# DLR-RM/AugmentedAutoencoder

Measured on NVIDIA H100. Metric: pose queries/sec (encode+codebook NN), higher is better.
Workload: dtype f32 via split-fp16 tensor-core products (3x, fp32 accumulate)

## Files before the change

### augmentedautoencoder_b200/csrc/tc_gemm.cu

```cuda
#include <limits.h>

#include <algorithm>
#include <vector>

#include "tc.cuh"
#include "tc_common.cuh"
#include "tc_plan.cuh"

namespace aae {

using namespace tc;

PFN_tmapEncodeTiled get_tmap_encoder() {
  static PFN_tmapEncodeTiled fn = nullptr;
  if (!fn) {
    void* p = nullptr;
    cudaDriverEntryPointQueryResult q;
    if (cudaGetDriverEntryPoint("cuTensorMapEncodeTiled", &p, cudaEnableDefault, &q) == cudaSuccess && q == cudaDriverEntryPointSuccess)
      fn = reinterpret_cast<PFN_tmapEncodeTiled>(p);
  }
  return fn;
}

int make_tmap_f16(CUtensorMap* out, const void* base, int rank, const uint64_t* dims, const uint64_t* strides_bytes, const uint32_t* box,
                  int swizzle_bytes) {
  PFN_tmapEncodeTiled enc = get_tmap_encoder();
  if (!enc) { set_error("cuTensorMapEncodeTiled is unavailable in this driver"); return AAE_ERR_CUDA; }
  cuuint64_t gdim[5], gstr[4];
  cuuint32_t bx[5], es[5];
  for (int i = 0; i < rank; ++i) { gdim[i] = dims[i]; bx[i] = box[i]; es[i] = 1; }
  for (int i = 0; i + 1 < rank; ++i) gstr[i] = strides_bytes[i];
  CUresult r = enc(out, CU_TENSOR_MAP_DATA_TYPE_FLOAT16, (cuuint32_t)rank, const_cast<void*>(base), gdim, gstr, bx, es,
                   CU_TENSOR_MAP_INTERLEAVE_NONE, swizzle_bytes == 64 ? CU_TENSOR_MAP_SWIZZLE_64B : CU_TENSOR_MAP_SWIZZLE_128B,
                   CU_TENSOR_MAP_L2_PROMOTION_L2_256B,
                   CU_TENSOR_MAP_FLOAT_OOB_FILL_NONE);
  if (r != CUDA_SUCCESS) { set_error("cuTensorMapEncodeTiled failed with CUresult %d (rank %d)", (int)r, rank); return AAE_ERR_CUDA; }
  return AAE_OK;
}

template <int N_TILE, int STAGES, int PLANES = 2>
struct TcSmem {
  static constexpr int A_BYTES = 128 * TC_KCH * 2;
  static constexpr int W_BYTES = N_TILE * TC_KCH * 2;
  static constexpr int STAGE_BYTES = PLANES * A_BYTES + PLANES * W_BYTES;
  static constexpr int BODY = STAGES * STAGE_BYTES;
  static constexpr int TOTAL = BODY + 1024  + 256 ;
};

struct TcTile {
  int m0, n0, z, it_begin, it_end;
};
template <int N_TILE>
__device__ __forceinline__ TcTile tc_tile(const TcGemmParams& p, const TcTiles& g, int t) {
  TcTile r;
  const int yz = t / g.n;
  const int y = yz % g.m;
  r.z = yz / g.m;
  r.m0 = y * 128;
  r.n0 = (t - yz * g.n) * N_TILE;
  r.it_begin = r.z * p.iters_per_split;
  r.it_end = min(p.taps * p.chunks_per_tap, r.it_begin + p.iters_per_split);
  return r;
}

template <int N_TILE, int STAGES, int PLANES = 2>
__global__ void __launch_bounds__(TC_THREADS, 1)
tc_gemm_kernel(const __grid_constant__ CUtensorMap tm_a_hi, const __grid_constant__ CUtensorMap tm_a_lo,
               const __grid_constant__ CUtensorMap tm_w_hi, const __grid_constant__ CUtensorMap tm_w_lo, const TcGemmParams p,
               const TcTiles tiles) {
  using S = TcSmem<N_TILE, STAGES, PLANES>;
  constexpr int R = N_TILE / 2;
  extern __shared__ uint8_t smem_raw[];
  uint8_t* smem = reinterpret_cast<uint8_t*>((reinterpret_cast<uintptr_t>(smem_raw) + 1023) & ~(uintptr_t)1023);
  uint64_t* full_bar = reinterpret_cast<uint64_t*>(smem + S::BODY);
  uint64_t* empty_bar = full_bar + STAGES;

  const int warp = threadIdx.x >> 5;
  const int lane = threadIdx.x & 31;

  if (threadIdx.x == 0) {
    prefetch_tmap(&tm_a_hi);
    if constexpr (PLANES == 2) prefetch_tmap(&tm_a_lo);
    prefetch_tmap(&tm_w_hi);
    if constexpr (PLANES == 2) prefetch_tmap(&tm_w_lo);
    for (int s = 0; s < STAGES; ++s) { mbar_init(&full_bar[s], 1); mbar_init(&empty_bar[s], 2); }
    fence_barrier_init();
  }
  __syncthreads();

  if (warp < 4) {
    setmaxnreg_dec<TC_PRODUCER_REGS>();
    if (warp == 0 && lane == 0) {
      const int hw = p.OH * p.OW;
      int i = 0;
      for (int t = blockIdx.x; t < tiles.count; t += gridDim.x) {
        const TcTile T = tc_tile<N_TILE>(p, tiles, t);
        const int b0 = T.m0 / hw, rem = T.m0 - b0 * hw;
        const int oh0 = rem / p.OW, ow0 = rem - oh0 * p.OW;
        for (int it = T.it_begin; it < T.it_end; ++it, ++i) {
          const int s = i % STAGES;
          const uint32_t ph = (uint32_t)(i / STAGES) & 1u;
          mbar_wait(&empty_bar[s], ph ^ 1u);
          const int tap = it / p.chunks_per_tap, cc = it - tap * p.chunks_per_tap;
          uint8_t* st = smem + s * S::STAGE_BYTES;
          mbar_arrive_expect_tx(&full_bar[s], S::STAGE_BYTES);
          const int c0 = p.tap_ch[tap] + cc * TC_KCH;
          const int x = ow0 + p.tap_dj[tap], y = oh0 + p.tap_di[tap];
          const int kcol = it * TC_KCH;
          tma_load_4d(st, &tm_a_hi, &full_bar[s], c0, x, y, b0);
          if constexpr (PLANES == 2) tma_load_4d(st + S::A_BYTES, &tm_a_lo, &full_bar[s], c0, x, y, b0);
          tma_load_2d(st + PLANES * S::A_BYTES, &tm_w_hi, &full_bar[s], kcol, T.n0);
          if constexpr (PLANES == 2) tma_load_2d(st + 2 * S::A_BYTES + S::W_BYTES, &tm_w_lo, &full_bar[s], kcol, T.n0);
        }
      }
    }
  } else {
    setmaxnreg_inc<TC_CONSUMER_REGS>();
    const int wg = (warp - 4) >> 2;
    const bool releases = (warp & 3) == 0 && lane == 0;
    constexpr int H = R / 8;
    float acc[R], crs[R], v[R];
#pragma unroll
    for (int j = 0; j < R; ++j) { acc[j] = 0.f; crs[j] = 0.f; v[j] = 0.f; }
    int pm0 = 0, pn0 = 0, pz = 0, half = 2;
    auto epilogue_half = [&](int h) {
      if (h == 0) tc_epilogue_frag<PLANES, 0, H>(p, v, pm0, pn0, pz, warp, lane);
      else tc_epilogue_frag<PLANES, H, 2 * H>(p, v, pm0, pn0, pz, warp, lane);
    };
    int i = 0;
    for (int t = blockIdx.x; t < tiles.count; t += gridDim.x) {
      const TcTile T = tc_tile<N_TILE>(p, tiles, t);
      for (int it = T.it_begin; it < T.it_end; ++it, ++i) {
        const int s = i % STAGES;
        mbar_wait(&full_bar[s], (uint32_t)(i / STAGES) & 1u);
        const uint32_t st = smem_u32(smem + s * S::STAGE_BYTES);
        const uint32_t a_off = (uint32_t)(wg * 64 * TC_KCH * 2);
        const uint64_t a_hi = make_sw128_kmajor_desc(st + a_off);
        const uint64_t a_lo = make_sw128_kmajor_desc(st + S::A_BYTES + a_off);
        const uint64_t w_hi = make_sw128_kmajor_desc(st + PLANES * S::A_BYTES);
        const uint64_t w_lo = make_sw128_kmajor_desc(st + 2 * S::A_BYTES + S::W_BYTES);
        wgmma_fence_regs(acc);
        if constexpr (PLANES == 2) wgmma_fence_regs(crs);
        wgmma_fence();
#pragma unroll
        for (int k = 0; k < TC_KCH / 16; ++k) {
          const uint32_t first = (it > T.it_begin || k > 0) ? 1u : 0u;
          Wgmma<N_TILE>::template ss<0, 0>(acc, desc_advance_k(a_hi, k), desc_advance_k(w_hi, k), first);
          if constexpr (PLANES == 2) {
            Wgmma<N_TILE>::template ss<0, 0>(crs, desc_advance_k(a_lo, k), desc_advance_k(w_hi, k), first);
            Wgmma<N_TILE>::template ss<0, 0>(crs, desc_advance_k(a_hi, k), desc_advance_k(w_lo, k), 1u);
          }
        }
        wgmma_commit();
        if (half < 2) epilogue_half(half++);
        wgmma_wait<1>();
        wgmma_fence_regs(acc);
        if constexpr (PLANES == 2) wgmma_fence_regs(crs);
        if (it > T.it_begin && releases) mbar_arrive(&empty_bar[(i - 1) % STAGES]);
      }
      wgmma_wait<0>();
      wgmma_fence_regs(acc);
      if constexpr (PLANES == 2) wgmma_fence_regs(crs);
      if (T.it_end > T.it_begin && releases) mbar_arrive(&empty_bar[(i - 1) % STAGES]);
      while (half < 2) epilogue_half(half++);
      tc_epilogue_values<PLANES>(p, acc, crs, T.it_end > T.it_begin, v);
      pm0 = T.m0 + wg * 64; pn0 = T.n0; pz = T.z; half = 0;
    }
    while (half < 2) epilogue_half(half++);
  }
}

namespace {

template <int PLANES>
__global__ void pack_weights_kernel(const float* __restrict__ w, int taps, int cin, int cout, float scale, __half* __restrict__ hi,
                                    __half* __restrict__ lo, unsigned* __restrict__ range_flag, unsigned range_bit) {
  __shared__ float tile[32][33];
  const int tap = blockIdx.z;
  const int ci0 = blockIdx.y * 32, co0 = blockIdx.x * 32;
  for (int i = threadIdx.y; i < 32; i += 8) {
    const int ci = ci0 + i, co = co0 + threadIdx.x;
    tile[i][threadIdx.x] = (ci < cin && co < cout) ? w[((long long)tap * cin + ci) * cout + co] : 0.f;
  }
  __syncthreads();
  for (int i = threadIdx.y; i < 32; i += 8) {
    const int co = co0 + i, ci = ci0 + threadIdx.x;
    if (co < cout && ci < cin)
      tc_store_f16<PLANES>(tile[threadIdx.x][i] * scale, hi, lo, (long long)co * taps * cin + (long long)tap * cin + ci, range_flag, range_bit);
  }
// ... 56 lines not shown
  return AAE_OK;
}

int TcPlanes::alloc(size_t n, int planes) {
  AAE_TRY(tc_dev_alloc((void**)&hi, n * sizeof(__half)));
  return planes == 2 ? tc_dev_alloc((void**)&lo, n * sizeof(__half)) : AAE_OK;
}

void TcPlanes::release() {
  cudaFree(hi);
  cudaFree(lo);
  hi = lo = nullptr;
}

int TcPlanes::encode(TcMaps& m, int rank, const uint64_t* dims, const uint64_t* strides_bytes, const uint32_t* box, int swizzle_bytes) const {
  AAE_TRY(make_tmap_f16(&m.hi, hi, rank, dims, strides_bytes, box, swizzle_bytes));
  if (lo == nullptr) {
    m.lo = m.hi;
    return AAE_OK;
  }
  return make_tmap_f16(&m.lo, lo, rank, dims, strides_bytes, box, swizzle_bytes);
}

constexpr int TC_STAGES_SPLIT = 3, TC_STAGES_FP16 = 6;
static_assert(TcSmem<TC_N_TILE, TC_STAGES_FP16, 1>::TOTAL == TcSmem<TC_N_TILE, TC_STAGES_SPLIT>::TOTAL, "same footprint");

int tc_launch_layer(const TcLayer& T, dim3 tiles, cudaStream_t s, int planes) {
  const long long count = (long long)tiles.x * tiles.y * tiles.z;
  AAE_REQUIRE(count <= INT_MAX, "tc_gemm: %lld tiles exceed the kernel's int tile index", count);
  int device = 0, sms = 0;
  AAE_CUDA_OK(cudaGetDevice(&device));
  AAE_CUDA_OK(cudaDeviceGetAttribute(&sms, cudaDevAttrMultiProcessorCount, device));
  const TcTiles g{(int)tiles.y, (int)tiles.x, (int)count};
  const unsigned ctas = (unsigned)std::min<long long>(count, sms);
  return with_planes(planes, [&](auto P) {
    constexpr int STAGES = P == 1 ? TC_STAGES_FP16 : TC_STAGES_SPLIT;
    using S = TcSmem<TC_N_TILE, STAGES, P>;
    auto kern = tc_gemm_kernel<TC_N_TILE, STAGES, P>;
    AAE_CUDA_OK(cudaFuncSetAttribute(kern, cudaFuncAttributeMaxDynamicSharedMemorySize, S::TOTAL));
    kern<<<ctas, TC_THREADS, S::TOTAL, s>>>(T.tm_a.hi, T.tm_a.lo, T.tm_w.hi, T.tm_w.lo, T.gp, g);
    AAE_LAUNCH_OK();
    return AAE_OK;
  });
}

int tc_encoder_create(int device, const aae_net_cfg* cfg, TcEncoder** out) {
  *out = nullptr;
  const int L = cfg->num_layers;
  AAE_REQUIRE(aae_device_supported(device), "AAE_PREC_TC_SPLIT needs a compute-capability 9.0 device (wgmma/TMA)");
  AAE_REQUIRE(L >= 2, "AAE_PREC_TC_SPLIT: at least two conv layers expected");
  const int planes = tc_planes(cfg->precision);
  if (planes == 1 && !tc_conv1_supported(cfg)) {
    set_error("AAE_PREC_TC_FP16: the first layer needs the tensor-core conv1 (128 x 128 x 3 crops, 128 filters, k = 5, stride 2)");
    return AAE_ERR_UNSUPPORTED;
  }
  TcEncoder* h = new TcEncoder();
  h->device = device;
  h->cfg = *cfg;
  h->planes = planes;
  int ih = (cfg->in_h + cfg->strides[0] - 1) / cfg->strides[0], iw = (cfg->in_w + cfg->strides[0] - 1) / cfg->strides[0], ic = cfg->filters[0];
  const int B = cfg->max_batch;
  int st = AAE_OK;
  for (int l = 1; l <= L && st == AAE_OK; ++l) {
// ... 3 lines not shown
    if (!dense) {
      if (cfg->strides[l] != 2 || cfg->kernel_size != 5 || (ih & 1) || (iw & 1) || ic % 64 != 0 || cfg->filters[l] % 32 != 0) {
        set_error("AAE_PREC_TC_SPLIT: layer %d unsupported (needs k=5, stride 2, even dims, Cin %% 64 == 0, Cout %% 32 == 0)", l);
        st = AAE_ERR_UNSUPPORTED;
        break;
      }
      T.in_h = ih; T.in_w = iw; T.in_c = ic;
      T.out_h = ih / 2; T.out_w = iw / 2; T.out_c = cfg->filters[l];
      T.taps = 25;
      if (!pow2(T.out_w) || !pow2(T.out_h) || T.out_w > 128) { set_error("AAE_PREC_TC_SPLIT: output dims must be powers of two <= 128"); st = AAE_ERR_UNSUPPORTED; break; }
      T.BW = T.out_w;
      T.BH = std::min(T.out_h, 128 / T.BW);
      T.BB = 128 / (T.BW * T.BH);
    } else {
      T.in_h = T.in_w = 1; T.in_c = ih * iw * ic;
      T.out_h = T.out_w = 1; T.out_c = cfg->latent;
      T.taps = 1; T.BW = 1; T.BH = 1; T.BB = 128;
      h->flat = T.in_c;
      if (T.in_c % 64 != 0 || T.out_c % 32 != 0) { set_error("AAE_PREC_TC_SPLIT: dense layer needs flat %% 64 == 0 and latent %% 32 == 0"); st = AAE_ERR_UNSUPPORTED; break; }
    }
    const int B_pad = (int)ceil_div(B, T.BB) * T.BB;
    if ((st = T.in.alloc((size_t)B_pad * T.in_h * T.in_w * T.in_c, planes)) != AAE_OK) break;
    if ((st = T.w.alloc((size_t)T.out_c * T.taps * T.in_c, planes)) != AAE_OK) break;
    if (!dense) {
      const uint64_t C4 = 4ull * T.in_c, W2 = T.in_w / 2, H2 = T.in_h / 2;
      const uint64_t dims[4] = {C4, W2, H2, (uint64_t)B_pad};
      const uint64_t strides[3] = {C4 * 2, W2 * C4 * 2, H2 * W2 * C4 * 2};
      const uint32_t box[4] = {(uint32_t)TC_KCH, (uint32_t)T.BW, (uint32_t)T.BH, (uint32_t)T.BB};
      if ((st = T.in.encode(T.tm_a, 4, dims, strides, box)) != AAE_OK) break;
    } else {
      const uint64_t dims[4] = {(uint64_t)T.in_c, 1, 1, (uint64_t)B_pad};
      const uint64_t strides[3] = {(uint64_t)T.in_c * 2, (uint64_t)T.in_c * 2, (uint64_t)T.in_c * 2};
      const uint32_t box[4] = {(uint32_t)TC_KCH, 1, 1, 128};
      if ((st = T.in.encode(T.tm_a, 4, dims, strides, box)) != AAE_OK) break;
    }
    {
      const uint64_t K = (uint64_t)T.taps * T.in_c;
      const uint64_t dims[2] = {K, (uint64_t)T.out_c};
      const uint64_t strides[1] = {K * 2};
      const uint32_t box[2] = {(uint32_t)TC_KCH, (uint32_t)std::min(TC_N_TILE, T.out_c)};
      if ((st = T.w.encode(T.tm_w, 2, dims, strides, box)) != AAE_OK) break;
    }
    TcGemmParams& g = T.gp;
    g.N = T.out_c; g.OH = T.out_h; g.OW = T.out_w; g.BW = T.BW; g.BH = T.BH;
    g.taps = T.taps; g.chunks_per_tap = T.in_c / TC_KCH;
    g.iters_per_split = g.taps * g.chunks_per_tap;
    for (int t = 0; t < T.taps; ++t) {
      if (dense) { g.tap_di[t] = 0; g.tap_dj[t] = 0; g.tap_ch[t] = 0; continue; }
      const int kh = t / 5, kw = t % 5;
      g.tap_di[t] = (int8_t)((kh + 1) / 2 - 1);
      g.tap_dj[t] = (int8_t)((kw + 1) / 2 - 1);
      g.tap_ch[t] = ((((kh + 1) & 1) << 1) | ((kw + 1) & 1)) * T.in_c;
    }
    g.unscale = 1.f / (ACT_SCALE * W_SCALE);
    g.out_scale = ACT_SCALE;
    g.relu = dense ? 0 : 1;
    h->layers.push_back(T);
    if (!dense) { ih = T.out_h; iw = T.out_w; ic = T.out_c; }
  }
  if (st == AAE_OK) {
    for (size_t i = 0; i + 1 < h->layers.size(); ++i) {
      TcGemmParams& g = h->layers[i].gp;
      g.out_hi = h->layers[i + 1].in.hi;
      g.out_lo = h->layers[i + 1].in.lo;
      g.out_mode = (i + 2 == h->layers.size()) ? OUT_PLAIN_SPLIT : OUT_S2D_SPLIT;
    }
    TcLayer& D = h->layers.back();
    const int total = D.gp.taps * D.gp.chunks_per_tap;
    h->dense_splits = std::min(total, 66);
    D.gp.iters_per_split = (total + h->dense_splits - 1) / h->dense_splits;
    h->dense_splits = (total + D.gp.iters_per_split - 1) / D.gp.iters_per_split;
    D.gp.out_mode = OUT_F32;
    st = dev_alloc((void**)&h->partials, (size_t)h->dense_splits * (B + 128) * cfg->latent * sizeof(float));
    D.gp.out_f32 = h->partials;
  }
  if (st == AAE_OK) st = dev_alloc((void**)&h->range_flag, sizeof(unsigned));
  if (st == AAE_OK)
    for (size_t i = 0; i + 1 < h->layers.size(); ++i) {
      h->layers[i].gp.range_flag = h->range_flag;
      h->layers[i].gp.range_bit = 1u << (i + 1);
    }
  if (st == AAE_OK && tc_conv1_supported(cfg)) st = tc_conv1_create(device, cfg, &h->conv1);
  if (st != AAE_OK) { tc_encoder_destroy(h); return st; }
  *out = h;
  return AAE_OK;
}

void tc_encoder_destroy(TcEncoder* h) {
  if (!h) return;
  for (auto& T : h->layers) { T.in.release(); T.w.release(); }
  cudaFree(h->partials);
  cudaFree(h->fwd_partials);
  cudaFree(h->dbg);
  if (h->owns_range_flag) cudaFree(h->range_flag);
// ... 62 lines not shown
    T.gp.M = dense ? B : B * T.out_h * T.out_w;
    dim3 grid((unsigned)ceil_div(T.gp.M, 128), (unsigned)ceil_div(T.out_c, TC_N_TILE), dense ? (unsigned)h->dense_splits : 1u);
    int splits = 1;
    if (!dense && T.gp.out_mode != OUT_F32) {
      const int tiles = (int)(grid.x * grid.y), total_iters = T.gp.taps * T.gp.chunks_per_tap;
      if (tiles * 2 <= 132) {
        splits = std::min(132 / tiles, std::max(1, total_iters / 24));
        const size_t per_split = (size_t)T.gp.M * T.gp.N;
        if (per_split * (size_t)splits > h->fwd_partial_floats) {
          const size_t want = std::min<size_t>(per_split * (size_t)splits, (size_t)32 << 20);
          if (want > h->fwd_partial_floats) {
            cudaFree(h->fwd_partials);
            h->fwd_partials = nullptr; h->fwd_partial_floats = 0;
            AAE_TRY(dev_alloc((void**)&h->fwd_partials, want * sizeof(float)));
            h->fwd_partial_floats = want;
          }
          splits = (int)std::min<size_t>((size_t)splits, h->fwd_partial_floats / per_split);
        }
        splits = std::max(splits, 1);
      }
    }
    if (splits > 1) {
      TcLayer S = T;
      const int total_iters = T.gp.taps * T.gp.chunks_per_tap;
      S.gp.iters_per_split = (int)ceil_div(total_iters, splits);
      splits = (int)ceil_div(total_iters, S.gp.iters_per_split);
      S.gp.out_mode = OUT_F32;
      S.gp.out_f32 = h->fwd_partials;
      grid.z = (unsigned)splits;
      AAE_TRY(tc_launch_layer(S, grid, s, h->planes));
      const long long groups = (long long)T.gp.M * (T.gp.N >> 3);
      const unsigned fin_grid = (unsigned)std::min<long long>(132 * 8, ceil_div(groups, 256));
      with_planes(h->planes, [&](auto P) { splitk_forward_finish_kernel<P><<<fin_grid, 256, 0, s>>>(h->fwd_partials, splits, T.gp); });
      AAE_LAUNCH_OK();
    } else {
      AAE_TRY(tc_launch_layer(T, grid, s, h->planes));
    }
    if (dense) AAE_TRY(launch_splitk_reduce(h->partials, h->dense_splits, (int64_t)B * cfg.latent, cfg.latent, dense_b, ACT_NONE, z_out, s));
    timer->mark(s);
  }
  return AAE_OK;
}

int tc_encoder_set_bias(TcEncoder* h, int layer, const float* bias_dev) {
  if (layer >= 1 && layer < (int)h->layers.size()) h->layers[layer - 1].gp.bias = bias_dev;
  return AAE_OK;
}

int tc_encoder_activation(TcEncoder* h, int layer, int B, const float** ptr, int64_t* count, cudaStream_t s) {
// ... 66 lines not shown
    }
    x[((b * 2 * h + 2 * i + (cls >> 1)) * (2LL * w) + 2 * j + (cls & 1)) * c + co] = 1.f / (1.f + expf(-s));
  }
}

__global__ void tile_bias_kernel(const float* __restrict__ b, int cout, float* __restrict__ out) {
  const int i = blockIdx.x * blockDim.x + threadIdx.x;
  if (i < 4 * cout) out[i] = b[i % cout];
}

}

int tc_layer_setup_plain(TcLayer& T, int B, int planes) {
  const int B_pad = (int)ceil_div(B, T.BB) * T.BB;
  const uint64_t K = (uint64_t)T.taps * T.in_c;
  const int rows = (int)ceil_div(T.gp.N, TC_N_TILE) * TC_N_TILE;
  AAE_TRY(T.in.alloc((size_t)B_pad * T.in_h * T.in_w * T.in_c, planes));
  AAE_TRY(T.w.alloc((size_t)rows * K, planes));
  {
    const uint64_t dims[4] = {(uint64_t)T.in_c, (uint64_t)T.in_w, (uint64_t)T.in_h, (uint64_t)B_pad};
    const uint64_t strides[3] = {(uint64_t)T.in_c * 2, (uint64_t)T.in_w * T.in_c * 2, (uint64_t)T.in_h * T.in_w * T.in_c * 2};
    const uint32_t box[4] = {(uint32_t)TC_KCH, (uint32_t)T.BW, (uint32_t)T.BH, (uint32_t)T.BB};
    AAE_TRY(T.in.encode(T.tm_a, 4, dims, strides, box));
  }
  const uint64_t dims[2] = {K, (uint64_t)rows};
  const uint64_t strides[1] = {K * 2};
  const uint32_t box[2] = {(uint32_t)TC_KCH, (uint32_t)TC_N_TILE};
  return T.w.encode(T.tm_w, 2, dims, strides, box);
}

int tc_decoder_create(int device, const aae_net_cfg* cfg, TcDecoder** out) {
  *out = nullptr;
  AAE_REQUIRE(aae_device_supported(device), "AAE_PREC_TC_SPLIT needs a compute-capability 9.0 device (wgmma/TMA)");
  const int L = cfg->num_layers;
  AAE_REQUIRE(cfg->kernel_size == 5 && cfg->in_h == cfg->in_w, "AAE_PREC_TC_SPLIT decoder: kernel 5, square crops");
  TcDecoder* h = new TcDecoder();
  h->device = device;
  h->cfg = *cfg;
  h->planes = tc_planes(cfg->precision);
  const int B = cfg->max_batch;
  int h0 = cfg->in_h;
  for (int i = 0; i < L; ++i) h0 /= 2;
  std::vector<int> nf(L);
  for (int i = 0; i < L; ++i) nf[i] = cfg->filters[L - 1 - i];
  int st = AAE_OK;
  for (int l = 0; l <= L && st == AAE_OK; ++l) {
// ... 8 lines not shown
    } else {
      const int hh = h0 << (l - 1);
      T.in_h = T.in_w = hh; T.in_c = nf[l - 1];
      const int cout = l < L ? nf[l] : cfg->in_c;
      T.out_h = T.out_w = 2 * hh; T.out_c = cout;
      T.taps = 9;
      if (hh > 128 || (hh & (hh - 1)) || T.in_c % 64 != 0 || (l < L && cout % 64 != 0)) {
        set_error("tc decoder: layer %d unsupported (power-of-two size <= 128, Cin %% 64, Cout %% 64)", l); st = AAE_ERR_UNSUPPORTED; break;
      }
      T.BW = hh; T.BH = std::min(hh, 128 / T.BW); T.BB = 128 / (T.BW * T.BH);
      g.OH = g.OW = hh;
      if (l < L) { g.N = 4 * cout; g.relu = 1; g.out_mode = OUT_D2S_SPLIT; }
      else {
        if (36 * cout > 128) {
          set_error("tc decoder: %d output channels, the tensor-core output layer takes at most 3 (AAE_PREC_FP32_SIMT takes any count)", cout);
          st = AAE_ERR_UNSUPPORTED; break;
        }
        T.taps = 1; g.N = 128; g.relu = 0; g.out_mode = OUT_F32;
        st = dev_alloc((void**)&h->out_p, (size_t)ceil_div((int64_t)B * hh * hh, 128) * 128 * 128 * sizeof(float));
        if (st != AAE_OK) break;
      }
    }
    g.BW = T.BW; g.BH = T.BH; g.taps = T.taps; g.chunks_per_tap = T.in_c / TC_KCH;
    g.iters_per_split = g.taps * g.chunks_per_tap;
    for (int t = 0; t < T.taps; ++t) {
      g.tap_di[t] = (int8_t)(T.taps == 1 ? 0 : t / 3 - 1);
      g.tap_dj[t] = (int8_t)(T.taps == 1 ? 0 : t % 3 - 1);
      g.tap_ch[t] = 0;
    }
    g.unscale = 1.f / (ACT_SCALE * W_SCALE);
    g.out_scale = ACT_SCALE;
    if ((st = tc_layer_setup_plain(T, B, h->planes)) != AAE_OK) { h->layers.push_back(T); break; }
    h->layers.push_back(T);
    float* bz = nullptr;
    if (l > 0 && l < L) st = dev_alloc((void**)&bz, (size_t)g.N * sizeof(float));
    h->bias_dev.push_back(bz);
    h->wm_floats = std::max(h->wm_floats, (size_t)9 * T.in_c * 4 * T.out_c);
  }
  if (st == AAE_OK) st = dev_alloc((void**)&h->wm_tmp, h->wm_floats * sizeof(float));
  if (st == AAE_OK) st = dev_alloc((void**)&h->range_flag, sizeof(unsigned));
  if (st == AAE_OK) {
    for (size_t i = 0; i + 1 < h->layers.size(); ++i) {
      h->layers[i].gp.out_hi = h->layers[i + 1].in.hi;
      h->layers[i].gp.out_lo = h->layers[i + 1].in.lo;
      h->layers[i].gp.range_flag = h->range_flag;
      h->layers[i].gp.range_bit = 1u << i;
    }
// ... 82 lines not shown
```

### augmentedautoencoder_b200/csrc/tc_plan.cuh

```cuda
#pragma once
#include <stdlib.h>

#include <type_traits>
#include <vector>

#include "tc.cuh"
#include "tc_common.cuh"

namespace aae {

enum TcOutMode : int {
  OUT_S2D_SPLIT = 0,
  OUT_PLAIN_SPLIT = 1,
  OUT_F32 = 2,
  OUT_D2S_SPLIT = 3
};

struct TcGemmParams {
  int M;
  int N;
  int OH, OW;
  int BW, BH;
  int taps;
  int chunks_per_tap;
  int iters_per_split;
  int8_t tap_di[32], tap_dj[32];
  int tap_ch[32];
  float unscale;
  const unsigned* amax_bits;
  float out_scale;
  const float* bias;
  int relu;
  int out_mode;
  __half* out_hi;
  __half* out_lo;
  float* out_f32;
  unsigned* range_flag;
  unsigned range_bit;
};

constexpr float TC_F16_OVERFLOW = 65520.f;



__host__ __device__ __forceinline__ int tc_dyn_exponent(unsigned amax_bits) {
  int e = (int)((amax_bits >> 23) & 0xffu) - 127;
  return e < -100 ? -100 : (e > 100 ? 100 : e);
}
__device__ __forceinline__ float tc_dyn_scale(unsigned amax_bits) { return __int_as_float((127 + 13 - tc_dyn_exponent(amax_bits)) << 23); }
__device__ __forceinline__ float tc_dyn_unscale(unsigned amax_bits) { return __int_as_float((127 - 13 + tc_dyn_exponent(amax_bits)) << 23); }

constexpr float ACT_SCALE = 16.f;
constexpr float W_SCALE = 256.f;
constexpr int TC_STAGES = 2;
constexpr int TC_THREADS = 384;
constexpr int TC_N_TILE = 128;
constexpr int TC_PRODUCER_REGS = 24, TC_CONSUMER_REGS = 240;
constexpr int TC_KCH = 64;

struct TcMaps {
  CUtensorMap hi, lo;
};

struct TcPlanes {
  __half* hi = nullptr;
  __half* lo = nullptr;
  int alloc(size_t n, int planes);
  void release();
  int encode(TcMaps& m, int rank, const uint64_t* dims, const uint64_t* strides_bytes, const uint32_t* box, int swizzle_bytes = 128) const;
};

template <class F>
auto with_planes(int planes, F&& f) {
  return planes == 1 ? f(std::integral_constant<int, 1>{}) : f(std::integral_constant<int, 2>{});
}

struct TcLayer {
  int in_h, in_w, in_c, out_h, out_w, out_c;
  int taps, BW, BH, BB;
  TcPlanes in;
  TcPlanes w;
  TcMaps tm_a, tm_w;
  TcGemmParams gp;
};

struct TcEncoder {
  int device;
  aae_net_cfg cfg;
  unsigned* range_flag = nullptr;
  bool owns_range_flag = true;
  std::vector<TcLayer> layers;
  int flat;
  float* partials = nullptr;
  float* fwd_partials = nullptr;
  size_t fwd_partial_floats = 0;
  int dense_splits = 1;
  TcConv1* conv1 = nullptr;
  int planes = 2;
  float* dbg = nullptr;
  size_t dbg_floats = 0;
};


struct TcDecoder {
  int device;
// ... 192 lines not shown
    for (int h = 0; h < 2; ++h) {
      const TcRow& r = rows[h];
      if (!r.valid) continue;
      float f[2] = {fmaxf(__fadd_rn(v[4 * j + 2 * h], b0), floor_v), fmaxf(__fadd_rn(v[4 * j + 2 * h + 1], b1), floor_v)};
      amax = fmaxf(amax, fmaxf(fabsf(f[0]), fabsf(f[1])));
      long long off = r.row_off + n;
      if (p.out_mode == OUT_D2S_SPLIT) {
        const int cls = n / cq, co = n - cls * cq;
        off = ((long long)(r.b * 2 * p.OH + 2 * r.i + (cls >> 1)) * (2 * p.OW) + 2 * r.j + (cls & 1)) * cq + co;
      }
      tc_store_f16<PLANES>(f, p.out_scale, p.out_hi, p.out_lo, off);
    }
  }
  if (p.range_flag != nullptr && !(amax * p.out_scale < TC_F16_OVERFLOW)) atomicOr(p.range_flag, p.range_bit);
}

struct TcTiles {
  int n, m, count;
};

int tc_launch_layer(const TcLayer& T, dim3 tiles, cudaStream_t s, int planes);
int tc_dev_alloc(void** p, size_t bytes);
int tc_layer_setup_plain(TcLayer& T, int B, int planes);

}
```

### augmentedautoencoder_b200/csrc/tc_train.cu

```cuda
#include <algorithm>
#include <vector>

#include "tc.cuh"
#include "tc_common.cuh"
#include "tc_plan.cuh"

namespace aae {

using namespace tc;

struct TcWgradParams {
  int cin_blocks;
  int OH, OW;
  int BWk, BHk;
  int chunks_per_image;
  int total_chunks;
  int chunks_per_split;
  int8_t tap_di[32], tap_dj[32];
  int tap_ch[32];
  int m_tiles;
  TcGemmParams ep;
};

template <int N_TILE, int STAGES, int PLANES = 2>
// ... 439 lines not shown
  AAE_REQUIRE(enc && dec && enc->conv1, "tensor-core trainer: needs the tensor-core encoder (incl. conv1) and decoder plans");
  AAE_REQUIRE(enc->planes == dec->planes, "tensor-core trainer: the encoder and decoder plans use different operand planes");
  TcTrainPlan* h = new TcTrainPlan();
  h->device = enc->device; h->max_batch = max_batch; h->enc = enc; h->dec = dec; h->planes = enc->planes;
  const int B = max_batch;
  int st = AAE_OK;
  const int Ld = (int)dec->layers.size() - 1;
  const int Le = (int)enc->layers.size() - 1;
  size_t raw_max = 0, part_max = 0, wm_max = 0;
  auto add_unit = [&](TcUnit& U, const TcLayer& F, int x_c_total) -> int {
    TcLayer& T = U.dg;
    memset(&T.gp, 0, sizeof(T.gp));
    T.in_h = U.gh; T.in_w = U.gw; T.in_c = U.gN;
    T.out_h = U.gh; T.out_w = U.gw; T.out_c = U.nd;
    T.taps = U.dg_taps;
    T.BW = U.gw; T.BH = std::min(U.gh, 128 / T.BW); T.BB = 128 / (T.BW * T.BH);
    if (U.gw > 128 || (U.gw & (U.gw - 1)) || (U.gh & (U.gh - 1)) || U.gN % TC_KCH != 0 || U.nd % TC_N_TILE != 0 || U.cin % 128 != 0 ||
        U.gN % 64 != 0 || (U.gh * U.gw) % 32 != 0) {
      set_error("tensor-core trainer: layer geometry unsupported (G %dx%dx%d, dgrad N %d, Cin %d)", U.gh, U.gw, U.gN, U.nd, U.cin);
      return AAE_ERR_UNSUPPORTED;
    }
    TcGemmParams& g = T.gp;
    g.N = U.nd; g.OH = U.gh; g.OW = U.gw; g.BW = T.BW; g.BH = T.BH;
    g.taps = T.taps; g.chunks_per_tap = U.gN / TC_KCH; g.iters_per_split = g.taps * g.chunks_per_tap;
    for (int t = 0; t < T.taps; ++t) {
      g.tap_di[t] = (int8_t)(T.taps == 1 ? 0 : t / 3 - 1);
      g.tap_dj[t] = (int8_t)(T.taps == 1 ? 0 : t % 3 - 1);
      g.tap_ch[t] = 0;
    }
    g.unscale = 1.f / W_SCALE;
    g.out_mode = OUT_F32;
    AAE_TRY(tc_layer_setup_plain(T, B, h->planes));
    U.x = F.in;
    const int x_bpad = (int)ceil_div(B, F.BB) * F.BB, g_bpad = (int)ceil_div(B, T.BB) * T.BB;
    AAE_TRY(make_wgrad_maps(U, x_c_total, x_bpad, g_bpad));
    for (int t = 0; t < U.taps_w; ++t) { U.wp.tap_di[t] = F.gp.tap_di[t]; U.wp.tap_dj[t] = F.gp.tap_dj[t]; U.wp.tap_ch[t] = F.gp.tap_ch[t]; }
    raw_max = std::max(raw_max, (size_t)B * U.gh * U.gw * U.nd);
    wm_max = std::max(wm_max, (size_t)U.taps_w * U.cin * U.gN);
    return AAE_OK;
  };
  for (int l = Ld; l >= 1 && st == AAE_OK; --l) {
    const TcLayer& F = dec->layers[l];
    TcUnit U;
    U.enc = false; U.cin = F.in_c; U.cout = F.out_c;
    U.gh = F.in_h; U.gw = F.in_w;
    U.sep = l == Ld;
    U.gN = U.sep ? 128 : 4 * F.out_c;
// ... 139 lines not shown

int tc_train_conv1_wgrad(TcTrainPlan* h, const float* x_dev, int B, float* dw_out, cudaStream_t s) {
  TcUnit& U = h->units[h->c1];
  const aae_net_cfg& cfg = h->enc->cfg;
  const long long pixels = (long long)B * U.gh * U.gw;
  const int pad_t = std::max((U.gh - 1) * 2 + 5 - cfg.in_h, 0) / 2, pad_l = std::max((U.gw - 1) * 2 + 5 - cfg.in_w, 0) / 2;
  with_planes(h->planes, [&](auto P) {
    conv1_im2col_kernel<P><<<ew_grid(pixels * 16), 256, 0, s>>>(x_dev, pixels, cfg.in_h, cfg.in_w, U.gh, U.gw, pad_t, pad_l, ACT_SCALE, h->c1_x.hi,
                                                                h->c1_x.lo);
  });
  AAE_LAUNCH_OK();
  AAE_REQUIRE((size_t)128 * U.gN <= h->wm_floats, "tc trainer: scratch too small for the conv1 wgrad");
  AAE_TRY(tc_train_unit_wgrad(h, h->c1, B, h->wm, s));
  AAE_CUDA_OK(cudaMemcpyAsync(dw_out, h->wm, (size_t)75 * U.gN * sizeof(float), cudaMemcpyDeviceToDevice, s));
  return AAE_OK;
}

int tc_train_unit_dgrad(TcTrainPlan* h, int u, int B, cudaStream_t s) {
  TcUnit& U = h->units[u];
  TcLayer& T = U.dg;
  T.gp.M = B * U.gh * U.gw;
  T.gp.amax_bits = h->amax + u;
  const int m_tiles = (int)ceil_div(T.gp.M, 128), n_tiles = U.nd / TC_N_TILE;
  const int total_iters = T.gp.taps * T.gp.chunks_per_tap;
  int splits = std::max(1, 132 / std::max(1, m_tiles * n_tiles));
  splits = std::min(splits, std::max(1, total_iters / 64));
  const long long mn = (long long)T.gp.M * U.nd;
  if ((size_t)splits * (size_t)mn > h->partial_floats) splits = 1;
  T.gp.iters_per_split = (int)ceil_div(total_iters, splits);
  splits = (int)ceil_div(total_iters, T.gp.iters_per_split);
  T.gp.out_f32 = splits > 1 ? h->partials : h->raw;
  dim3 grid((unsigned)m_tiles, (unsigned)n_tiles, (unsigned)splits);
  AAE_TRY(tc_launch_layer(T, grid, s, h->planes));
  if (splits > 1) AAE_TRY(launch_splitk_reduce(h->partials, splits, mn, U.nd, nullptr, ACT_NONE, h->raw, s));
  return AAE_OK;
}

int tc_train_finish(TcTrainPlan* h, int u, int next, int B, bool keep_masked, float* db_out, cudaStream_t s) {
  TcUnit& U = h->units[u];
  const long long groups = (long long)B * U.gh * U.gw * U.nd / 8;
  __half *hi = nullptr, *lo = nullptr;
  unsigned* slot = nullptr;
  if (next >= 0) {
    TcUnit& Nx = h->units[next];
    AAE_REQUIRE((long long)Nx.gh * Nx.gw * Nx.gN == (long long)U.gh * U.gw * U.nd, "tc trainer: unit %d does not feed unit %d", u, next);
    hi = Nx.dg.in.hi; lo = Nx.dg.in.lo; slot = h->amax + next;
    amax_kernel<<<ew_grid(groups), 256, 0, s>>>(h->raw, U.mask_hi, groups, slot);
    AAE_LAUNCH_OK();
  }
  const int mode = U.enc ? REMAP_S2D_TO_PLAIN : (next >= 0 ? REMAP_PLAIN_TO_S2D : REMAP_SAME);
  const int C = U.enc ? U.cin : U.nd;
  const int gpr = U.nd / 8;
  const unsigned grid = db_out ? std::min(ew_grid(groups), 132u * 4u) : ew_grid(groups);
// ... 32 lines not shown
```

Before: 37750.

## Share halo A tiles across vertical conv taps with separate A and W rings

Splits the TMA pipeline into an A ring and a weight ring. Taps that share channel offset and horizontal shift are grouped, so one taller halo box of activations is loaded once and reused by the vertically shifted taps through row offsets into the shared-memory descriptor. This cuts redundant activation loads per conv tap. In exchange it adds group-planning logic, extra barriers and a larger A footprint, and it changes the split-K unit accounting.

After: 39030 (median of 6 runs). 1.03x the previous value.

```diff
diff --git a/augmentedautoencoder_b200/csrc/tc_gemm.cu b/augmentedautoencoder_b200/csrc/tc_gemm.cu
--- a/augmentedautoencoder_b200/csrc/tc_gemm.cu
+++ b/augmentedautoencoder_b200/csrc/tc_gemm.cu
@@ -38,17 +38,16 @@
   return AAE_OK;
 }
 
-template <int N_TILE, int STAGES, int PLANES = 2>
+template <int N_TILE, int W_STAGES, int PLANES = 2>
 struct TcSmem {
-  static constexpr int A_BYTES = 128 * TC_KCH * 2;
   static constexpr int W_BYTES = N_TILE * TC_KCH * 2;
-  static constexpr int STAGE_BYTES = PLANES * A_BYTES + PLANES * W_BYTES;
-  static constexpr int BODY = STAGES * STAGE_BYTES;
+  static constexpr int W_STAGE_BYTES = PLANES * W_BYTES;
+  static constexpr int BODY = TC_A_RING_BYTES + W_STAGES * W_STAGE_BYTES;
   static constexpr int TOTAL = BODY + 1024  + 256 ;
 };
 
 struct TcTile {
-  int m0, n0, z, it_begin, it_end;
+  int m0, n0, z, u_begin, u_end;
 };
 template <int N_TILE>
 __device__ __forceinline__ TcTile tc_tile(const TcGemmParams& p, const TcTiles& g, int t) {
@@ -58,22 +57,26 @@
   r.z = yz / g.m;
   r.m0 = y * 128;
   r.n0 = (t - yz * g.n) * N_TILE;
-  r.it_begin = r.z * p.iters_per_split;
-  r.it_end = min(p.taps * p.chunks_per_tap, r.it_begin + p.iters_per_split);
+  r.u_begin = r.z * p.units_per_split;
+  r.u_end = min(p.groups * p.chunks_per_tap, r.u_begin + p.units_per_split);
   return r;
 }
 
-template <int N_TILE, int STAGES, int PLANES = 2>
+template <int N_TILE, int W_STAGES, int PLANES = 2>
 __global__ void __launch_bounds__(TC_THREADS, 1)
 tc_gemm_kernel(const __grid_constant__ CUtensorMap tm_a_hi, const __grid_constant__ CUtensorMap tm_a_lo,
                const __grid_constant__ CUtensorMap tm_w_hi, const __grid_constant__ CUtensorMap tm_w_lo, const TcGemmParams p,
                const TcTiles tiles) {
-  using S = TcSmem<N_TILE, STAGES, PLANES>;
+  using S = TcSmem<N_TILE, W_STAGES, PLANES>;
   constexpr int R = N_TILE / 2;
   extern __shared__ uint8_t smem_raw[];
   uint8_t* smem = reinterpret_cast<uint8_t*>((reinterpret_cast<uintptr_t>(smem_raw) + 1023) & ~(uintptr_t)1023);
-  uint64_t* full_bar = reinterpret_cast<uint64_t*>(smem + S::BODY);
-  uint64_t* empty_bar = full_bar + STAGES;
+  uint64_t* a_full = reinterpret_cast<uint64_t*>(smem + S::BODY);
+  uint64_t* a_empty = a_full + TC_A_SLOTS_MAX;
+  uint64_t* w_full = a_empty + TC_A_SLOTS_MAX;
+  uint64_t* w_empty = w_full + W_STAGES;
+  uint8_t* w_ring = smem + TC_A_RING_BYTES;
+  const int a_plane = p.a_rows * TC_KCH * 2, a_slot = PLANES * a_plane;
 
   const int warp = threadIdx.x >> 5;
   const int lane = threadIdx.x & 31;
@@ -83,7 +86,8 @@
     if constexpr (PLANES == 2) prefetch_tmap(&tm_a_lo);
     prefetch_tmap(&tm_w_hi);
     if constexpr (PLANES == 2) prefetch_tmap(&tm_w_lo);
-    for (int s = 0; s < STAGES; ++s) { mbar_init(&full_bar[s], 1); mbar_init(&empty_bar[s], 2); }
+    for (int s = 0; s < p.a_slots; ++s) { mbar_init(&a_full[s], 1); mbar_init(&a_empty[s], 2); }
+    for (int s = 0; s < W_STAGES; ++s) { mbar_init(&w_full[s], 1); mbar_init(&w_empty[s], 2); }
     fence_barrier_init();
   }
   __syncthreads();
@@ -92,25 +96,31 @@
     setmaxnreg_dec<TC_PRODUCER_REGS>();
     if (warp == 0 && lane == 0) {
       const int hw = p.OH * p.OW;
-      int i = 0;
+      int ia = 0, iw = 0;
       for (int t = blockIdx.x; t < tiles.count; t += gridDim.x) {
         const TcTile T = tc_tile<N_TILE>(p, tiles, t);
         const int b0 = T.m0 / hw, rem = T.m0 - b0 * hw;
         const int oh0 = rem / p.OW, ow0 = rem - oh0 * p.OW;
-        for (int it = T.it_begin; it < T.it_end; ++it, ++i) {
-          const int s = i % STAGES;
-          const uint32_t ph = (uint32_t)(i / STAGES) & 1u;
-          mbar_wait(&empty_bar[s], ph ^ 1u);
-          const int tap = it / p.chunks_per_tap, cc = it - tap * p.chunks_per_tap;
-          uint8_t* st = smem + s * S::STAGE_BYTES;
-          mbar_arrive_expect_tx(&full_bar[s], S::STAGE_BYTES);
-          const int c0 = p.tap_ch[tap] + cc * TC_KCH;
-          const int x = ow0 + p.tap_dj[tap], y = oh0 + p.tap_di[tap];
-          const int kcol = it * TC_KCH;
-          tma_load_4d(st, &tm_a_hi, &full_bar[s], c0, x, y, b0);
-          if constexpr (PLANES == 2) tma_load_4d(st + S::A_BYTES, &tm_a_lo, &full_bar[s], c0, x, y, b0);
-          tma_load_2d(st + PLANES * S::A_BYTES, &tm_w_hi, &full_bar[s], kcol, T.n0);
-          if constexpr (PLANES == 2) tma_load_2d(st + 2 * S::A_BYTES + S::W_BYTES, &tm_w_lo, &full_bar[s], kcol, T.n0);
+        for (int u = T.u_begin; u < T.u_end; ++u, ++ia) {
+          const int g = u / p.chunks_per_tap, cc = u - g * p.chunks_per_tap;
+          const int sa = ia & (p.a_slots - 1);
+          mbar_wait(&a_empty[sa], (ia & p.a_slots) ? 0u : 1u);
+          uint8_t* a = smem + sa * a_slot;
+          mbar_arrive_expect_tx(&a_full[sa], a_slot);
+          const int c0 = p.grp_ch[g] + cc * TC_KCH;
+          const int x = ow0 + p.grp_dx[g], y = oh0 + p.grp_dy[g];
+          tma_load_4d(a, &tm_a_hi, &a_full[sa], c0, x, y, b0);
+          if constexpr (PLANES == 2) tma_load_4d(a + a_plane, &tm_a_lo, &a_full[sa], c0, x, y, b0);
+          const int first = p.grp_first[g], ntaps = p.grp_ntaps[g];
+          for (int k = 0; k < ntaps; ++k, ++iw) {
+            const int sw = iw % W_STAGES;
+            mbar_wait(&w_empty[sw], ((uint32_t)(iw / W_STAGES) & 1u) ^ 1u);
+            uint8_t* w = w_ring + sw * S::W_STAGE_BYTES;
+            mbar_arrive_expect_tx(&w_full[sw], S::W_STAGE_BYTES);
+            const int kcol = (p.grp_tap[first + k] * p.chunks_per_tap + cc) * TC_KCH;
+            tma_load_2d(w, &tm_w_hi, &w_full[sw], kcol, T.n0);
+            if constexpr (PLANES == 2) tma_load_2d(w + S::W_BYTES, &tm_w_lo, &w_full[sw], kcol, T.n0);
+          }
         }
       }
     }
@@ -122,49 +132,64 @@
     float acc[R], crs[R], v[R];
 #pragma unroll
     for (int j = 0; j < R; ++j) { acc[j] = 0.f; crs[j] = 0.f; v[j] = 0.f; }
-    int pm0 = 0, pn0 = 0, pz = 0, half = 2;
+    int pt = 0, half = 2;
     auto epilogue_half = [&](int h) {
-      if (h == 0) tc_epilogue_frag<PLANES, 0, H>(p, v, pm0, pn0, pz, warp, lane);
-      else tc_epilogue_frag<PLANES, H, 2 * H>(p, v, pm0, pn0, pz, warp, lane);
+      const TcTile P = tc_tile<N_TILE>(p, tiles, pt);
+      if (h == 0) tc_epilogue_frag<PLANES, 0, H>(p, v, P.m0 + wg * 64, P.n0, P.z, warp, lane);
+      else tc_epilogue_frag<PLANES, H, 2 * H>(p, v, P.m0 + wg * 64, P.n0, P.z, warp, lane);
     };
-    int i = 0;
+    int ia = 0, iw = 0;
     for (int t = blockIdx.x; t < tiles.count; t += gridDim.x) {
       const TcTile T = tc_tile<N_TILE>(p, tiles, t);
-      for (int it = T.it_begin; it < T.it_end; ++it, ++i) {
-        const int s = i % STAGES;
-        mbar_wait(&full_bar[s], (uint32_t)(i / STAGES) & 1u);
-        const uint32_t st = smem_u32(smem + s * S::STAGE_BYTES);
-        const uint32_t a_off = (uint32_t)(wg * 64 * TC_KCH * 2);
-        const uint64_t a_hi = make_sw128_kmajor_desc(st + a_off);
-        const uint64_t a_lo = make_sw128_kmajor_desc(st + S::A_BYTES + a_off);
-        const uint64_t w_hi = make_sw128_kmajor_desc(st + PLANES * S::A_BYTES);
-        const uint64_t w_lo = make_sw128_kmajor_desc(st + 2 * S::A_BYTES + S::W_BYTES);
-        wgmma_fence_regs(acc);
-        if constexpr (PLANES == 2) wgmma_fence_regs(crs);
-        wgmma_fence();
+      for (int u = T.u_begin; u < T.u_end; ++u, ++ia) {
+        const int g = u / p.chunks_per_tap;
+        const int sa = ia & (p.a_slots - 1);
+        mbar_wait(&a_full[sa], (ia & p.a_slots) ? 1u : 0u);
+        const int first = p.grp_first[g], ntaps = p.grp_ntaps[g];
+        for (int k = 0; k < ntaps; ++k, ++iw) {
+          const int sw = iw % W_STAGES;
+          mbar_wait(&w_full[sw], (uint32_t)(iw / W_STAGES) & 1u);
+          const uint32_t a_tap = smem_u32(smem + sa * a_slot) + (uint32_t)((wg * p.a_wg_rows + p.grp_row[first + k]) * TC_KCH * 2);
+          const uint32_t st = smem_u32(w_ring + sw * S::W_STAGE_BYTES);
+          const uint64_t a_hi = make_sw128_kmajor_desc(a_tap);
+          const uint64_t a_lo = make_sw128_kmajor_desc(a_tap + (uint32_t)a_plane);
+          const uint64_t w_hi = make_sw128_kmajor_desc(st);
+          const uint64_t w_lo = make_sw128_kmajor_desc(st + S::W_BYTES);
+          const bool accumulate = u > T.u_begin || k > 0;
+          wgmma_fence_regs(acc);
+          if constexpr (PLANES == 2) wgmma_fence_regs(crs);
+          wgmma_fence();
 #pragma unroll
-        for (int k = 0; k < TC_KCH / 16; ++k) {
-          const uint32_t first = (it > T.it_begin || k > 0) ? 1u : 0u;
-          Wgmma<N_TILE>::template ss<0, 0>(acc, desc_advance_k(a_hi, k), desc_advance_k(w_hi, k), first);
-          if constexpr (PLANES == 2) {
-            Wgmma<N_TILE>::template ss<0, 0>(crs, desc_advance_k(a_lo, k), desc_advance_k(w_hi, k), first);
-            Wgmma<N_TILE>::template ss<0, 0>(crs, desc_advance_k(a_hi, k), desc_advance_k(w_lo, k), 1u);
+          for (int kk = 0; kk < TC_KCH / 16; ++kk) {
+            const uint32_t scale_d = (accumulate || kk > 0) ? 1u : 0u;
+            Wgmma<N_TILE>::template ss<0, 0>(acc, desc_advance_k(a_hi, kk), desc_advance_k(w_hi, kk), scale_d);
+            if constexpr (PLANES == 2) {
+              Wgmma<N_TILE>::template ss<0, 0>(crs, desc_advance_k(a_lo, kk), desc_advance_k(w_hi, kk), scale_d);
+              Wgmma<N_TILE>::template ss<0, 0>(crs, desc_advance_k(a_hi, kk), desc_advance_k(w_lo, kk), 1u);
+            }
+          }
+          wgmma_commit();
+          if (half < 2) epilogue_half(half++);
+          wgmma_wait<1>();
+          wgmma_fence_regs(acc);
+          if constexpr (PLANES == 2) wgmma_fence_regs(crs);
+          if (accumulate && releases) {
+            mbar_arrive(&w_empty[(iw - 1) % W_STAGES]);
+            if (k == 0) mbar_arrive(&a_empty[(ia - 1) & (p.a_slots - 1)]);
           }
         }
-        wgmma_commit();
-        if (half < 2) epilogue_half(half++);
-        wgmma_wait<1>();
-        wgmma_fence_regs(acc);
-        if constexpr (PLANES == 2) wgmma_fence_regs(crs);
-        if (it > T.it_begin && releases) mbar_arrive(&empty_bar[(i - 1) % STAGES]);
       }
       wgmma_wait<0>();
       wgmma_fence_regs(acc);
       if constexpr (PLANES == 2) wgmma_fence_regs(crs);
-      if (T.it_end > T.it_begin && releases) mbar_arrive(&empty_bar[(i - 1) % STAGES]);
+      const bool has_work = T.u_end > T.u_begin;
+      if (has_work && releases) {
+        mbar_arrive(&w_empty[(iw - 1) % W_STAGES]);
+        mbar_arrive(&a_empty[(ia - 1) & (p.a_slots - 1)]);
+      }
       while (half < 2) epilogue_half(half++);
-      tc_epilogue_values<PLANES>(p, acc, crs, T.it_end > T.it_begin, v);
-      pm0 = T.m0 + wg * 64; pn0 = T.n0; pz = T.z; half = 0;
+      tc_epilogue_values<PLANES>(p, acc, crs, has_work, v);
+      pt = t; half = 0;
     }
     while (half < 2) epilogue_half(half++);
   }
@@ -267,23 +292,74 @@
   return make_tmap_f16(&m.lo, lo, rank, dims, strides_bytes, box, swizzle_bytes);
 }
 
-constexpr int TC_STAGES_SPLIT = 3, TC_STAGES_FP16 = 6;
-static_assert(TcSmem<TC_N_TILE, TC_STAGES_FP16, 1>::TOTAL == TcSmem<TC_N_TILE, TC_STAGES_SPLIT>::TOTAL, "same footprint");
+constexpr int TC_W_STAGES_SPLIT = 3, TC_W_STAGES_FP16 = 6;
+static_assert(TcSmem<TC_N_TILE, TC_W_STAGES_FP16, 1>::TOTAL == TcSmem<TC_N_TILE, TC_W_STAGES_SPLIT>::TOTAL, "same footprint");
+static_assert(TcSmem<TC_N_TILE, TC_W_STAGES_SPLIT>::TOTAL <= 227 * 1024, "tc_gemm_kernel: shared memory over the sm_90 limit");
+
+int tc_plan_groups(TcLayer& T, int planes, const uint64_t* dims, const uint64_t* strides_bytes) {
+  TcGemmParams& g = T.gp;
+  AAE_REQUIRE(g.taps >= 1 && g.taps <= 32, "tc plan: %d taps (at most 32)", g.taps);
+  AAE_REQUIRE(T.BW * T.BH * T.BB == 128, "tc plan: box %d x %d x %d is not one 128-row tile", T.BW, T.BH, T.BB);
+  const int halo_rows = (T.BH + 2) * T.BW * T.BB;
+  bool halo = g.taps > 1 && T.BW % 8 == 0 && (T.BB == 1 || (T.BB == 2 && T.BH * T.BW == 64)) &&
+              2 * planes * halo_rows * TC_KCH * 2 <= TC_A_RING_BYTES && T.BH + 2 <= 256;
+  for (int t = 0; t < g.taps; ++t) halo = halo && g.tap_di[t] >= -1 && g.tap_di[t] <= 1;
+  g.groups = 0;
+  for (int t = 0; t < g.taps; ++t) {
+    int grp = -1;
+    for (int q = 0; halo && q < g.groups; ++q)
+      if (g.grp_ch[q] == g.tap_ch[t] && g.grp_dx[q] == g.tap_dj[t]) grp = q;
+    if (grp < 0) {
+      grp = g.groups++;
+      g.grp_ch[grp] = g.tap_ch[t];
+      g.grp_dx[grp] = g.tap_dj[t];
+      g.grp_dy[grp] = (int8_t)(halo ? -1 : g.tap_di[t]);
+      g.grp_ntaps[grp] = 0;
+    }
+    g.grp_ntaps[grp]++;
+  }
+  int n = 0;
+  for (int q = 0; q < g.groups; ++q) {
+    g.grp_first[q] = (int8_t)n;
+    for (int t = 0; t < g.taps; ++t) {
+      if (halo ? (g.grp_ch[q] != g.tap_ch[t] || g.grp_dx[q] != g.tap_dj[t]) : t != q) continue;
+      g.grp_tap[n] = (int8_t)t;
+      g.grp_row[n] = (int16_t)(halo ? (g.tap_di[t] + 1) * T.BW : 0);
+      ++n;
+    }
+  }
+  AAE_REQUIRE(n == g.taps, "tc plan: tap groups cover %d of %d taps", n, g.taps);
+  g.a_rows = halo ? halo_rows : 128;
+  g.a_wg_rows = halo && T.BB == 2 ? (T.BH + 2) * T.BW : 64;
+  const int slot_bytes = planes * g.a_rows * TC_KCH * 2;
+  g.a_slots = 1;
+  while (2 * g.a_slots <= TC_A_SLOTS_MAX && 2 * g.a_slots * slot_bytes <= TC_A_RING_BYTES) g.a_slots *= 2;
+  AAE_REQUIRE(g.a_slots >= 2, "tc plan: an A slot of %d bytes leaves fewer than two in the ring", slot_bytes);
+  AAE_REQUIRE(g.a_rows % 8 == 0 && g.a_wg_rows % 8 == 0, "tc plan: A box rows %d / warpgroup offset %d off the 8-row atom", g.a_rows, g.a_wg_rows);
+  for (int i = 0; i < n; ++i) AAE_REQUIRE(g.grp_row[i] % 8 == 0 && g.grp_row[i] + g.a_wg_rows + 64 <= g.a_rows, "tc plan: tap row %d outside the A box", g.grp_row[i]);
+  g.units_per_split = g.groups * g.chunks_per_tap;
+  if (!halo) return AAE_OK;
+  const uint32_t box[4] = {(uint32_t)TC_KCH, (uint32_t)T.BW, (uint32_t)(T.BH + 2), (uint32_t)T.BB};
+  return T.in.encode(T.tm_halo, 4, dims, strides_bytes, box);
+}
 
 int tc_launch_layer(const TcLayer& T, dim3 tiles, cudaStream_t s, int planes) {
   const long long count = (long long)tiles.x * tiles.y * tiles.z;
   AAE_REQUIRE(count <= INT_MAX, "tc_gemm: %lld tiles exceed the kernel's int tile index", count);
+  AAE_REQUIRE(T.gp.a_slots >= 2 && T.gp.a_slots <= TC_A_SLOTS_MAX && (T.gp.a_slots & (T.gp.a_slots - 1)) == 0 &&
+              T.gp.a_slots * planes * T.gp.a_rows * TC_KCH * 2 <= TC_A_RING_BYTES, "tc_gemm: layer without a tap-group plan");
   int device = 0, sms = 0;
   AAE_CUDA_OK(cudaGetDevice(&device));
   AAE_CUDA_OK(cudaDeviceGetAttribute(&sms, cudaDevAttrMultiProcessorCount, device));
   const TcTiles g{(int)tiles.y, (int)tiles.x, (int)count};
   const unsigned ctas = (unsigned)std::min<long long>(count, sms);
+  const TcMaps& a = T.gp.a_rows == 128 ? T.tm_a : T.tm_halo;
   return with_planes(planes, [&](auto P) {
-    constexpr int STAGES = P == 1 ? TC_STAGES_FP16 : TC_STAGES_SPLIT;
-    using S = TcSmem<TC_N_TILE, STAGES, P>;
-    auto kern = tc_gemm_kernel<TC_N_TILE, STAGES, P>;
+    constexpr int W_STAGES = P == 1 ? TC_W_STAGES_FP16 : TC_W_STAGES_SPLIT;
+    using S = TcSmem<TC_N_TILE, W_STAGES, P>;
+    auto kern = tc_gemm_kernel<TC_N_TILE, W_STAGES, P>;
     AAE_CUDA_OK(cudaFuncSetAttribute(kern, cudaFuncAttributeMaxDynamicSharedMemorySize, S::TOTAL));
-    kern<<<ctas, TC_THREADS, S::TOTAL, s>>>(T.tm_a.hi, T.tm_a.lo, T.tm_w.hi, T.tm_w.lo, T.gp, g);
+    kern<<<ctas, TC_THREADS, S::TOTAL, s>>>(a.hi, a.lo, T.tm_w.hi, T.tm_w.lo, T.gp, g);
     AAE_LAUNCH_OK();
     return AAE_OK;
   });
@@ -333,17 +409,20 @@
     const int B_pad = (int)ceil_div(B, T.BB) * T.BB;
     if ((st = T.in.alloc((size_t)B_pad * T.in_h * T.in_w * T.in_c, planes)) != AAE_OK) break;
     if ((st = T.w.alloc((size_t)T.out_c * T.taps * T.in_c, planes)) != AAE_OK) break;
+    uint64_t a_dims[4], a_strides[3];
     if (!dense) {
       const uint64_t C4 = 4ull * T.in_c, W2 = T.in_w / 2, H2 = T.in_h / 2;
       const uint64_t dims[4] = {C4, W2, H2, (uint64_t)B_pad};
       const uint64_t strides[3] = {C4 * 2, W2 * C4 * 2, H2 * W2 * C4 * 2};
-      const uint32_t box[4] = {(uint32_t)TC_KCH, (uint32_t)T.BW, (uint32_t)T.BH, (uint32_t)T.BB};
-      if ((st = T.in.encode(T.tm_a, 4, dims, strides, box)) != AAE_OK) break;
+      memcpy(a_dims, dims, sizeof(dims)); memcpy(a_strides, strides, sizeof(strides));
     } else {
       const uint64_t dims[4] = {(uint64_t)T.in_c, 1, 1, (uint64_t)B_pad};
       const uint64_t strides[3] = {(uint64_t)T.in_c * 2, (uint64_t)T.in_c * 2, (uint64_t)T.in_c * 2};
-      const uint32_t box[4] = {(uint32_t)TC_KCH, 1, 1, 128};
-      if ((st = T.in.encode(T.tm_a, 4, dims, strides, box)) != AAE_OK) break;
+      memcpy(a_dims, dims, sizeof(dims)); memcpy(a_strides, strides, sizeof(strides));
+    }
+    {
+      const uint32_t box[4] = {(uint32_t)TC_KCH, (uint32_t)T.BW, (uint32_t)T.BH, (uint32_t)T.BB};
+      if ((st = T.in.encode(T.tm_a, 4, a_dims, a_strides, box)) != AAE_OK) break;
     }
     {
       const uint64_t K = (uint64_t)T.taps * T.in_c;
@@ -355,7 +434,6 @@
     TcGemmParams& g = T.gp;
     g.N = T.out_c; g.OH = T.out_h; g.OW = T.out_w; g.BW = T.BW; g.BH = T.BH;
     g.taps = T.taps; g.chunks_per_tap = T.in_c / TC_KCH;
-    g.iters_per_split = g.taps * g.chunks_per_tap;
     for (int t = 0; t < T.taps; ++t) {
       if (dense) { g.tap_di[t] = 0; g.tap_dj[t] = 0; g.tap_ch[t] = 0; continue; }
       const int kh = t / 5, kw = t % 5;
@@ -363,6 +441,7 @@
       g.tap_dj[t] = (int8_t)((kw + 1) / 2 - 1);
       g.tap_ch[t] = ((((kh + 1) & 1) << 1) | ((kw + 1) & 1)) * T.in_c;
     }
+    if ((st = tc_plan_groups(T, planes, a_dims, a_strides)) != AAE_OK) break;
     g.unscale = 1.f / (ACT_SCALE * W_SCALE);
     g.out_scale = ACT_SCALE;
     g.relu = dense ? 0 : 1;
@@ -377,10 +456,10 @@
       g.out_mode = (i + 2 == h->layers.size()) ? OUT_PLAIN_SPLIT : OUT_S2D_SPLIT;
     }
     TcLayer& D = h->layers.back();
-    const int total = D.gp.taps * D.gp.chunks_per_tap;
+    const int total = D.gp.groups * D.gp.chunks_per_tap;
     h->dense_splits = std::min(total, 66);
-    D.gp.iters_per_split = (total + h->dense_splits - 1) / h->dense_splits;
-    h->dense_splits = (total + D.gp.iters_per_split - 1) / D.gp.iters_per_split;
+    D.gp.units_per_split = (total + h->dense_splits - 1) / h->dense_splits;
+    h->dense_splits = (total + D.gp.units_per_split - 1) / D.gp.units_per_split;
     D.gp.out_mode = OUT_F32;
     st = dev_alloc((void**)&h->partials, (size_t)h->dense_splits * (B + 128) * cfg->latent * sizeof(float));
     D.gp.out_f32 = h->partials;
@@ -489,9 +568,9 @@
     }
     if (splits > 1) {
       TcLayer S = T;
-      const int total_iters = T.gp.taps * T.gp.chunks_per_tap;
-      S.gp.iters_per_split = (int)ceil_div(total_iters, splits);
-      splits = (int)ceil_div(total_iters, S.gp.iters_per_split);
+      const int total_units = T.gp.groups * T.gp.chunks_per_tap;
+      S.gp.units_per_split = (int)ceil_div(total_units, splits);
+      splits = (int)ceil_div(total_units, S.gp.units_per_split);
       S.gp.out_mode = OUT_F32;
       S.gp.out_f32 = h->fwd_partials;
       grid.z = (unsigned)splits;
@@ -604,6 +683,7 @@
     const uint64_t strides[3] = {(uint64_t)T.in_c * 2, (uint64_t)T.in_w * T.in_c * 2, (uint64_t)T.in_h * T.in_w * T.in_c * 2};
     const uint32_t box[4] = {(uint32_t)TC_KCH, (uint32_t)T.BW, (uint32_t)T.BH, (uint32_t)T.BB};
     AAE_TRY(T.in.encode(T.tm_a, 4, dims, strides, box));
+    AAE_TRY(tc_plan_groups(T, planes, dims, strides));
   }
   const uint64_t dims[2] = {K, (uint64_t)rows};
   const uint64_t strides[1] = {K * 2};
@@ -658,7 +738,6 @@
       }
     }
     g.BW = T.BW; g.BH = T.BH; g.taps = T.taps; g.chunks_per_tap = T.in_c / TC_KCH;
-    g.iters_per_split = g.taps * g.chunks_per_tap;
     for (int t = 0; t < T.taps; ++t) {
       g.tap_di[t] = (int8_t)(T.taps == 1 ? 0 : t / 3 - 1);
       g.tap_dj[t] = (int8_t)(T.taps == 1 ? 0 : t % 3 - 1);
diff --git a/augmentedautoencoder_b200/csrc/tc_plan.cuh b/augmentedautoencoder_b200/csrc/tc_plan.cuh
--- a/augmentedautoencoder_b200/csrc/tc_plan.cuh
+++ b/augmentedautoencoder_b200/csrc/tc_plan.cuh
@@ -23,9 +23,17 @@
   int BW, BH;
   int taps;
   int chunks_per_tap;
-  int iters_per_split;
+  int units_per_split;
   int8_t tap_di[32], tap_dj[32];
   int tap_ch[32];
+  int groups;
+  int a_rows;
+  int a_wg_rows;
+  int a_slots;
+  int grp_ch[32];
+  int8_t grp_dy[32], grp_dx[32], grp_first[32], grp_ntaps[32];
+  int8_t grp_tap[32];
+  int16_t grp_row[32];
   float unscale;
   const unsigned* amax_bits;
   float out_scale;
@@ -57,6 +65,7 @@
 constexpr int TC_N_TILE = 128;
 constexpr int TC_PRODUCER_REGS = 24, TC_CONSUMER_REGS = 240;
 constexpr int TC_KCH = 64;
+constexpr int TC_A_RING_BYTES = 128 * 1024, TC_A_SLOTS_MAX = 8;
 
 struct TcMaps {
   CUtensorMap hi, lo;
@@ -81,6 +90,7 @@
   TcPlanes in;
   TcPlanes w;
   TcMaps tm_a, tm_w;
+  TcMaps tm_halo;
   TcGemmParams gp;
 };
 
@@ -319,5 +329,6 @@
 int tc_launch_layer(const TcLayer& T, dim3 tiles, cudaStream_t s, int planes);
 int tc_dev_alloc(void** p, size_t bytes);
 int tc_layer_setup_plain(TcLayer& T, int B, int planes);
-
-}
+int tc_plan_groups(TcLayer& T, int planes, const uint64_t* dims, const uint64_t* strides_bytes);
+
+}
diff --git a/augmentedautoencoder_b200/csrc/tc_train.cu b/augmentedautoencoder_b200/csrc/tc_train.cu
--- a/augmentedautoencoder_b200/csrc/tc_train.cu
+++ b/augmentedautoencoder_b200/csrc/tc_train.cu
@@ -485,7 +485,7 @@
     }
     TcGemmParams& g = T.gp;
     g.N = U.nd; g.OH = U.gh; g.OW = U.gw; g.BW = T.BW; g.BH = T.BH;
-    g.taps = T.taps; g.chunks_per_tap = U.gN / TC_KCH; g.iters_per_split = g.taps * g.chunks_per_tap;
+    g.taps = T.taps; g.chunks_per_tap = U.gN / TC_KCH;
     for (int t = 0; t < T.taps; ++t) {
       g.tap_di[t] = (int8_t)(T.taps == 1 ? 0 : t / 3 - 1);
       g.tap_dj[t] = (int8_t)(T.taps == 1 ? 0 : t % 3 - 1);
@@ -671,13 +671,13 @@
   T.gp.M = B * U.gh * U.gw;
   T.gp.amax_bits = h->amax + u;
   const int m_tiles = (int)ceil_div(T.gp.M, 128), n_tiles = U.nd / TC_N_TILE;
-  const int total_iters = T.gp.taps * T.gp.chunks_per_tap;
+  const int total_iters = T.gp.taps * T.gp.chunks_per_tap, total_units = T.gp.groups * T.gp.chunks_per_tap;
   int splits = std::max(1, 132 / std::max(1, m_tiles * n_tiles));
   splits = std::min(splits, std::max(1, total_iters / 64));
   const long long mn = (long long)T.gp.M * U.nd;
   if ((size_t)splits * (size_t)mn > h->partial_floats) splits = 1;
-  T.gp.iters_per_split = (int)ceil_div(total_iters, splits);
-  splits = (int)ceil_div(total_iters, T.gp.iters_per_split);
+  T.gp.units_per_split = (int)ceil_div(total_units, splits);
+  splits = (int)ceil_div(total_units, T.gp.units_per_split);
   T.gp.out_f32 = splits > 1 ? h->partials : h->raw;
   dim3 grid((unsigned)m_tiles, (unsigned)n_tiles, (unsigned)splits);
   AAE_TRY(tc_launch_layer(T, grid, s, h->planes));
```
